# FengDushuo/BBBP-Multi-Modal-Deep-Ensemble-Framework

Hardware: AMD Instinct MI355X
Metric: molecules/sec fwd+bwd (3-branch ensemble, B=512) (higher is better)
Workload: dtype f32; 1 GPU; MixedInputModel F=167 (MACCS) + 3x128x128 image, 6-layer encoder + 2-stage CNN + fusion + BN head; forward + MSE + backward + fused AdamW, train mode (dropout 0.1); global_batch=512, per_gpu_batch=512, parallelism=dp1, input=device-resident

## Files before the change

### bbbp-multi-modal-deep-ensemble-framework_amd/_lib.py

```python
from __future__ import annotations

import ctypes
import os
import re
from ctypes import (POINTER, Structure, c_char_p, c_double, c_float, c_int, c_long, c_size_t, c_uint8, c_uint64, c_void_p)

_HERE = os.path.dirname(os.path.abspath(__file__))
LIB_PATH = os.environ.get("BBBP_LIB", os.path.join(_HERE, "libbbbp_hip.so"))
HEADER_PATH = os.path.join(os.path.dirname(_HERE), "include", "bbbp_hip.h")

_lib = None


class MixedDesc(Structure):
    _fields_ = [("batch", c_int), ("fingerprint_size", c_int), ("nhead", c_int), ("num_layers", c_int),
                ("dim_feedforward", c_int), ("training", c_int), ("dropout_p", c_float), ("seed", c_uint64),
                ("need_input_grad", c_int), ("fusion", c_int), ("inference", c_int),
                ("world", c_int), ("rank", c_int), ("collective", c_void_p), ("collective_ctx", c_void_p)]


CollectiveFn = ctypes.CFUNCTYPE(c_int, c_void_p, c_int, c_int, c_int, ctypes.c_size_t, ctypes.c_size_t, ctypes.c_size_t, c_void_p)


class GemmDesc(Structure):
    _fields_ = [("transA", c_int), ("transB", c_int), ("M", c_int), ("N", c_int), ("K", c_int), ("alpha", c_float),
                ("A", c_void_p), ("lda", c_int), ("B", c_void_p), ("ldb", c_int), ("C", c_void_p), ("ldc", c_int),
                ("bias", c_void_p), ("residual", c_void_p), ("ldr", c_int), ("act", c_int),
                ("gate", c_void_p), ("ldg", c_int), ("gate_scale", c_float), ("batch", c_int),
                ("strideA", c_long), ("strideB", c_long), ("strideC", c_long), ("strideR", c_long), ("strideG", c_long),
                ("gate_after_residual", c_int), ("asum", c_void_p), ("drop_p", c_float), ("drop_seed", c_uint64)]


class MlpModel(Structure):
    _fields_ = [("n_layers", c_int), ("units", c_int * 5), ("activation", c_int), ("batch_size", c_int), ("n_train", c_int),
                ("n_iter_no_change", c_int), ("max_iter", c_int),
                ("lr_init", ctypes.c_double), ("alpha", ctypes.c_double), ("beta1", ctypes.c_double), ("beta2", ctypes.c_double),
                ("eps", ctypes.c_double), ("tol", ctypes.c_double),
                ("params", c_void_p), ("adam_m", c_void_p), ("adam_v", c_void_p), ("grads", c_void_p),
                ("act", c_void_p), ("delta", c_void_p), ("order", c_void_p), ("loss_curve", c_void_p),
                ("t", c_long), ("best_loss", ctypes.c_double), ("no_improve", c_int), ("n_iter", c_int), ("done", c_int)]


class GemmF64cDesc(Structure):
    _fields_ = [("layout", c_int), ("M", c_int), ("N", c_int), ("K", c_int),
                ("A", c_void_p), ("a_dtype", c_int), ("lda", c_long), ("B", c_void_p), ("b_dtype", c_int), ("ldb", c_long),
                ("a_shift", c_void_p), ("b_shift", c_void_p), ("row_scale", c_void_p),
                ("C", c_void_p), ("c_dtype", c_int), ("ldc", c_long), ("symmetric", c_int), ("split_k", c_int)]


class KnnDesc(Structure):
    _fields_ = [("m", c_int), ("n", c_int), ("d", c_int), ("k", c_int),
                ("Q", c_void_p), ("q_dtype", c_int), ("ldq", c_long), ("T", c_void_p), ("t_dtype", c_int), ("ldt", c_long),
                ("mu", c_void_p), ("q_norm", c_void_p), ("t_norm", c_void_p), ("dist", c_void_p), ("ind", c_void_p),
                ("exclude_self", c_int), ("slices", c_int)]


_FP = c_void_p
_PP = POINTER(c_void_p)

_SIGNATURES = {
    "bbbp_abi_version": (c_int, []),
    "bbbp_last_error": (c_char_p, []),
    "bbbp_gemm_workspace_bytes": (c_size_t, [c_int, c_int, c_int, c_int]),
    "bbbp_gemm_f32": (c_int, [c_void_p, c_int, c_int, c_int, c_int, c_int, c_float, _FP, c_int, _FP, c_int, _FP, c_int,
                              _FP, _FP, c_int, c_int, c_int, c_long, c_long, c_long, c_long, c_void_p, c_size_t]),
    "bbbp_gemm_folds_asum": (c_int, [c_int, c_int, c_int, c_int]),
    "bbbp_gemm_f32_grouped": (c_int, [c_void_p, POINTER(GemmDesc), c_int, c_void_p, c_size_t]),
    "bbbp_mixed_backward_wait_bucket": (c_int, [c_void_p, c_int]),
    "bbbp_mixed_backward_wait_released": (c_int, [c_void_p, c_int]),
    "bbbp_set_release_events": (c_int, [c_int]),
    "bbbp_mixed_bucket_param": (c_int, [POINTER(MixedDesc), c_int]),
    "bbbp_mixed_bucket_range": (c_int, [POINTER(MixedDesc), c_int, POINTER(c_int), POINTER(c_int)]),
    "bbbp_mixed_debug_ffn_gate": (c_int, [c_void_p, POINTER(MixedDesc), c_void_p, c_int, c_void_p]),
    "bbbp_mixed_debug_pool_mask": (c_int, [c_void_p, POINTER(MixedDesc), c_void_p, c_int, c_void_p]),
    "bbbp_set_graphs": (c_int, [c_int]),
    "bbbp_set_fused_head_bwd": (c_int, [c_int]),
    "bbbp_set_fused_encoder": (c_int, [c_int]),
    "bbbp_set_fold_outproj": (c_int, [c_int]),
    "bbbp_set_flash_attention": (c_int, [c_int]),
    "bbbp_set_gemm_split_bf16": (c_int, [c_int]),
    "bbbp_set_gemm_fold_reduce": (c_int, [c_int]),
    "bbbp_gemm_split_bf16_phases": (c_int, [POINTER(c_uint64)]),
    "bbbp_gbt_predict": (c_int, [c_void_p, c_void_p, c_long, c_int, c_void_p, c_void_p, c_void_p, c_void_p, c_void_p, c_void_p, c_int, c_float,
                         c_void_p, c_void_p]),
    "bbbp_oblivious_predict": (c_int, [c_void_p, c_void_p, c_long, c_int, c_void_p, c_void_p, c_void_p, c_void_p, c_void_p, c_void_p, c_int,
                               c_double, c_double, c_void_p, c_void_p]),
    "bbbp_linear_layernorm_supported": (c_int, [c_int, c_int, c_int]),
    "bbbp_linear_layernorm_fwd": (c_int, [c_void_p, c_void_p, c_int, c_void_p, c_void_p, c_void_p, c_int, c_void_p, c_int, c_void_p, c_int, c_void_p,
                                  c_void_p, c_void_p, c_void_p, c_int, c_int, c_int, c_float, c_float, c_uint64]),
    "bbbp_layernorm_linear_supported": (c_int, [c_int, c_int, c_int]),
    "bbbp_layernorm_linear_fwd": (c_int, [c_void_p, c_void_p, c_int, c_void_p, c_void_p, c_float, c_void_p, c_void_p, c_void_p, c_int, c_int, c_float,
                                  c_uint64, c_void_p, c_int, c_void_p, c_void_p, c_int, c_int, c_int]),
    "bbbp_forest_groups": (c_int, [c_int]),
    "bbbp_forest_predict": (c_int, [c_void_p, c_void_p, c_long, c_int, c_void_p, c_void_p, c_void_p, c_void_p, c_void_p, c_void_p, c_int,
                                    c_void_p, c_void_p]),
    "bbbp_mlp_train_epochs": (c_int, [c_void_p, c_void_p, c_int, c_void_p, c_void_p, c_int, c_int]),
    "bbbp_mlp_predict_proba": (c_int, [c_void_p, c_void_p, c_int, c_void_p, c_int, c_int, c_int, c_void_p]),
    "bbbp_pca_col_mean": (c_int, [c_void_p, c_void_p, c_int, c_long, c_int, c_long, c_void_p]),
    "bbbp_gemm_f64c_workspace_bytes": (c_size_t, [POINTER(GemmF64cDesc)]),
    "bbbp_gemm_f64c": (c_int, [c_void_p, POINTER(GemmF64cDesc), c_void_p, c_size_t]),
    "bbbp_knn_row_norms": (c_int, [c_void_p, c_void_p, c_int, c_long, c_int, c_long, c_void_p, c_void_p, c_void_p]),
    "bbbp_knn_workspace_bytes": (c_size_t, [POINTER(KnnDesc)]),
    "bbbp_knn_f64": (c_int, [c_void_p, POINTER(KnnDesc), c_void_p, c_size_t]),
    "bbbp_knn_vote": (c_int, [c_void_p, c_void_p, c_void_p, c_long, c_int, c_int, c_void_p, c_long, c_int, c_int, c_void_p, c_void_p]),
    "bbbp_graph_stats": (c_int, [POINTER(c_long), POINTER(c_long)]),
    "bbbp_conv_last_clock": (c_int, [POINTER(c_uint64), POINTER(c_uint64)]),
    "bbbp_set_conv_winograd": (c_int, [c_int]),
    "bbbp_get_conv_winograd": (c_int, []),
    "bbbp_conv_winograd_phases": (c_int, [POINTER(c_uint64)]),
    "bbbp_conv_b3_phases": (c_int, [POINTER(c_uint64)]),
    "bbbp_conv3x3_workspace_bytes": (c_size_t, [c_int, c_int, c_int, c_int, c_int]),
    "bbbp_conv3x3_relu_pool_fwd": (c_int, [c_void_p, _FP, _FP, _FP, _FP, c_void_p, c_int, c_int, c_int, c_int, c_int,
                                           c_void_p, c_size_t]),
    "bbbp_conv3x3_relu_pool_bwd_data": (c_int, [c_void_p, _FP, c_void_p, _FP, _FP, c_int, c_int, c_int, c_int, c_int,
                                                c_void_p, c_size_t]),
    "bbbp_conv3x3_relu_pool_bwd_weight": (c_int, [c_void_p, _FP, _FP, c_void_p, _FP, _FP, c_int, c_int, c_int, c_int,
                                                  c_int, c_void_p, c_size_t]),
    "bbbp_layernorm_fwd": (c_int, [c_void_p, _FP, _FP, _FP, _FP, _FP, _FP, _FP, c_int, c_int, c_float, c_float, c_uint64]),
    "bbbp_layernorm_bwd": (c_int, [c_void_p, _FP, _FP, _FP, _FP, _FP, _FP, _FP, _FP, _FP, c_int, c_int, c_float, c_uint64]),
    "bbbp_softmax_fwd": (c_int, [c_void_p, _FP, _FP, c_long, c_int, c_float, c_uint64]),
# ... 77 lines not shown
```

### bbbp-multi-modal-deep-ensemble-framework_amd/csrc/gemm.hip

```cpp
#include "common.h"
#include "bbbp_hip.h"
#include <mutex>
#include <type_traits>
#include <unordered_map>

#define TRY_RC(expr) do { int _rc = (expr); if (_rc) return _rc; } while (0)

typedef float f32x4u __attribute__((ext_vector_type(4), aligned(4)));
typedef float f32x2u __attribute__((ext_vector_type(2), aligned(4)));

namespace {

constexpr int bk_of(int tile) { return tile == 64 ? 16 : 32; }

struct GemmParams {
    const float* A; const float* B; float* C;
    const float* bias; const float* R;
    int M, N, K;
    int lda, ldb, ldc, ldr;
    long sA, sB, sC, sR;
    float alpha;
    int act;
    int splits, kchunk;
    float* slab;
// ... 237 lines not shown
            step = B3_BK;
        }
    }
    __device__ __forceinline__ void load(int set) {
#pragma unroll
        for (int i = 0; i < 4; ++i) { raw[set][i] = *reinterpret_cast<const f32x4u*>(ptr[i]); ptr[i] += step; }
        kpos += B3_BK;
    }
    __device__ __forceinline__ void load_tail(int set) {
        if constexpr (KMAJ) {
#pragma unroll
            for (int j = 0; j < 4; ++j) {
                const bool ok = kpos + j < kend;
                const f32x4u v = *reinterpret_cast<const f32x4u*>(ok ? ptr[j] : X0);
                raw[set][j] = ok ? v : f32x4u{0.f, 0.f, 0.f, 0.f};
            }
        } else {
            const int nv = kend - kpos;
#pragma unroll
            for (int i = 0; i < 4; ++i) {
                const float* q = nv > 0 ? ptr[i] : X0;
                f32x4u v;
#pragma unroll
                for (int e = 0; e < 4; ++e) { const float x = q[e < nv ? e : 0]; v[e] = e < nv ? x : 0.f; }
                raw[set][i] = v;
            }
        }
        kpos += B3_BK;
    }
    __device__ __forceinline__ void split(int set) {
#pragma unroll
        for (int i = 0; i < 4; ++i) {
            uint32_t h0, m0, l0, h1, m1, l1;
            if constexpr (KMAJ) {
                split2(raw[set][0][i], raw[set][1][i], h0, m0, l0);
                split2(raw[set][2][i], raw[set][3][i], h1, m1, l1);
            } else {
                split2(raw[set][i][0], raw[set][i][1], h0, m0, l0);
                split2(raw[set][i][2], raw[set][i][3], h1, m1, l1);
            }
            pk[i][0] = u32x2{h0, h1}; pk[i][1] = u32x2{m0, m1}; pk[i][2] = u32x2{l0, l1};
        }
    }
    __device__ __forceinline__ void store(uint16_t* dst) const {
#pragma unroll
        for (int i = 0; i < 4; ++i)
#pragma unroll
            for (int pl = 0; pl < 3; ++pl) *reinterpret_cast<u32x2*>(dst + soff[i] + pl * B3_PLANE) = pk[i][pl];
    }
};

__device__ unsigned long long g_gemm_b3_phase[7];

template <int LAYOUT, bool PROBE>
__device__ __forceinline__ void gemm_b3_body(const GemmParams& p) {
    BBBP_HIGH_PRIO();
    unsigned long long ph[5] = {0, 0, 0, 0, 0}, c0 = 0;
    const unsigned long long cyc_begin = PROBE ? __builtin_readcyclecounter() : 0, wall_begin = PROBE ? wall_clock64() : 0;
    constexpr bool A_KMAJ = (LAYOUT == 2), B_KMAJ = (LAYOUT != 0);
    extern __shared__ __attribute__((aligned(16))) uint16_t smem16[];
    uint16_t* As = smem16;
    uint16_t* Bs = smem16 + 3 * B3_PLANE;
    const int t = threadIdx.x, lane = t & 63, wave = t >> 6, r = lane & 31, h = lane >> 5;
    const int wm = wave >> 1, wn = wave & 1;
    const int batch = blockIdx.z / p.splits, split = blockIdx.z % p.splits;
    const int m0 = blockIdx.y * 128, n0 = blockIdx.x * 128;
    const int kbeg = split * p.kchunk;
    const int kend = min(p.K, kbeg + p.kchunk);
    const int nt = (kend - kbeg + B3_BK - 1) / B3_BK;
    const int tail_stage = ((kend - kbeg) % B3_BK) ? nt - 1 : -1;

    B3Loader<A_KMAJ> la;
    B3Loader<B_KMAJ> lb;
    la.init(p.A + (long)batch * p.sA, p.lda, p.M, m0, kbeg, kend, t);
    lb.init(p.B + (long)batch * p.sB, p.ldb, p.N, n0, kbeg, kend, t);
    auto load_stage = [&](int stage, int set) __attribute__((always_inline)) {
        if (stage == tail_stage) { la.load_tail(set); lb.load_tail(set); }
        else { la.load(set); lb.load(set); }
    };

    f32x16 acc[2][2];
#pragma unroll
    for (int i = 0; i < 2; ++i)
#pragma unroll
        for (int j = 0; j < 2; ++j)
#pragma unroll
            for (int q = 0; q < 16; ++q) acc[i][j][q] = 0.f;

    if (nt > 0) {
        load_stage(0, 0);
        if (nt > 1) load_stage(1, 1);
        la.split(0); lb.split(0);
        la.store(As); lb.store(Bs);
    }
    __syncthreads();
    const uint16_t* afrag = As + (wm * 64 + r) * B3_LD + 8 * h;
    const uint16_t* bfrag = Bs + (wn * 64 + r) * B3_LD + 8 * h;
    for (int it = 0; it < nt; it += 2) {
#pragma unroll
        for (int u = 0; u < 2; ++u) {
            const int cur = it + u;
            if (cur >= nt) break;
            if (PROBE) c0 = __builtin_readcyclecounter();
            if (cur + 2 < nt) load_stage(cur + 2, u);
            if (PROBE) { const unsigned long long c = __builtin_readcyclecounter(); ph[0] += c - c0; c0 = c; }
#pragma unroll
// ... 44 lines not shown
#pragma unroll
            for (int j = 0; j < 2; ++j) {
                const int n = n0 + wn * 64 + j * 32 + r;
#pragma unroll
                for (int q = 0; q < 16; ++q) {
                    const int m = m0 + wm * 64 + i * 32 + mfma_row(q, lane);
                    if (m < p.M && n < p.N) {
                        if (p.arrivals) __hip_atomic_store(&S[(long)m * p.N + n], acc[i][j][q], __ATOMIC_RELAXED, __HIP_MEMORY_SCOPE_AGENT);
                        else S[(long)m * p.N + n] = acc[i][j][q];
                    }
                }
            }
        if (!p.arrivals) return;
        __shared__ int s_last;
        asm volatile("s_waitcnt vmcnt(0)" ::: "memory");
        __syncthreads();
        if (t == 0) {
            unsigned* cnt = p.arrivals + ((long)batch * gridDim.y + blockIdx.y) * gridDim.x + blockIdx.x;
            const unsigned old = __hip_atomic_fetch_add(cnt, 1u, __ATOMIC_RELAXED, __HIP_MEMORY_SCOPE_AGENT);
            s_last = (old == (unsigned)p.splits - 1u) ? 1 : 0;
            if (s_last) __hip_atomic_store(cnt, 0u, __ATOMIC_RELAXED, __HIP_MEMORY_SCOPE_AGENT);
        }
        __syncthreads();
        if (!s_last) return;
        const long mn = (long)p.M * p.N;
        const float* S0 = p.slab + (long)batch * p.splits * mn;
        float* Cf = p.C + (long)batch * p.sC;
        const float* Rf = p.R ? p.R + (long)batch * p.sR : nullptr;
        const int tw = min(128, p.N - n0), th = min(128, p.M - m0);
        for (int e = t; e < th * 128; e += 256) {
            const int lm = e >> 7, ln = e & 127;
            if (ln >= tw) continue;
            const int m = m0 + lm, n = n0 + ln;
            const float* sp = S0 + (long)m * p.N + n;
            float sum = 0.f;
            int k = 0;
            for (; k + 8 <= p.splits; k += 8) {
                float v[8];
#pragma unroll
                for (int u = 0; u < 8; ++u) v[u] = __hip_atomic_load(sp + (long)(k + u) * mn, __ATOMIC_RELAXED, __HIP_MEMORY_SCOPE_AGENT);
#pragma unroll
                for (int u = 0; u < 8; ++u) sum += v[u];
            }
            for (; k < p.splits; ++k) sum += __hip_atomic_load(sp + (long)k * mn, __ATOMIC_RELAXED, __HIP_MEMORY_SCOPE_AGENT);
            float v = apply_act(p.alpha * sum + (p.bias ? p.bias[n] : 0.f), p.act);
            const float gsel = p.gate ? (p.gate[(long)batch * p.sG + (long)m * p.ldg + n] > 0.f ? p.gate_scale : 0.f) : 1.f;
            if (!p.gate_after) v *= gsel;
            if (Rf) v += Rf[(long)m * p.ldr + n];
            if (p.gate_after) v *= gsel;
            Cf[(long)m * p.ldc + n] = v;
        }
        return;
    }
    float* C = p.C + (long)batch * p.sC;
    const float* R = p.R ? p.R + (long)batch * p.sR : nullptr;
#pragma unroll
    for (int i = 0; i < 2; ++i)
#pragma unroll
        for (int j = 0; j < 2; ++j) {
            const int n = n0 + wn * 64 + j * 32 + r;
            const float bv = (p.bias && n < p.N) ? p.bias[n] : 0.f;
#pragma unroll
            for (int q = 0; q < 16; ++q) {
                const int m = m0 + wm * 64 + i * 32 + mfma_row(q, lane);
                if (m < p.M && n < p.N) {
                    float v = apply_act(p.alpha * acc[i][j][q] + bv, p.act);
                    const float gsel = p.gate ? (p.gate[(long)batch * p.sG + (long)m * p.ldg + n] > 0.f ? p.gate_scale : 0.f) : 1.f;
                    if (!p.gate_after) v *= gsel;
                    if (R) v += R[(long)m * p.ldr + n];
                    if (p.gate_after) v *= gsel;
                    C[(long)m * p.ldc + n] = v;
                }
            }
        }
}

template <int LAYOUT>
__global__ __launch_bounds__(256, 2) void gemm_b3_kernel(GemmParams p) { gemm_b3_body<LAYOUT, false>(p); }
template <int LAYOUT>
__global__ __launch_bounds__(256, 2) void gemm_b3_probe_kernel(GemmParams p) { gemm_b3_body<LAYOUT, true>(p); }

constexpr int B3S_T = 64;
#ifndef BBBP_B3S_DEPTH_NT
#define BBBP_B3S_DEPTH_NT 2
#endif
#ifndef BBBP_B3S_DEPTH_NN
#define BBBP_B3S_DEPTH_NN 2
#endif
constexpr int B3S_DEPTH_NT = BBBP_B3S_DEPTH_NT, B3S_DEPTH_NN = BBBP_B3S_DEPTH_NN;
constexpr int B3S_PLANE = B3S_T * B3_LD;
constexpr size_t B3S_LDS = (size_t)6 * B3S_PLANE * sizeof(uint16_t);

template <bool KMAJ, int SETS>
struct B3SLoader {
    static constexpr int NL = KMAJ ? 4 : 2;
    const float* ptr[NL];
    const float* X0;
    long step;
    int kpos, kend;
    int soff[NL];
    bool live;
    f32x4u raw[SETS][NL];
    u32x2 pk[NL][3];
    __device__ __forceinline__ void init(const float* X, int ld, int extent, int row0, int kbeg, int kend_, int t) {
        const int kq = t & 7, rq = t >> 3;
        X0 = X; kpos = kbeg + 4 * kq; kend = kend_;
        if constexpr (KMAJ) {
            live = rq < 16;
            const int cq = rq & 15;
            const int col = min(row0 + 4 * cq, extent - 4);
#pragma unroll
            for (int j = 0; j < 4; ++j) { ptr[j] = X + (long)(kbeg + 4 * kq + j) * ld + col; soff[j] = (4 * cq + j) * B3_LD + 4 * kq; }
            step = (long)B3_BK * ld;
        } else {
            live = true;
            const int a = rq & 3, b = rq >> 2;
            const int row = (b >> 2) * 16 + (b & 3) + 4 * a;
#pragma unroll
            for (int i = 0; i < 2; ++i) {
                ptr[i] = X + (long)min(row0 + row + 32 * i, extent - 1) * ld + kbeg + 4 * kq;
                soff[i] = (row + 32 * i) * B3_LD + 4 * kq;
            }
            step = B3_BK;
        }
    }
    __device__ __forceinline__ void load(int set) {
#pragma unroll
        for (int i = 0; i < NL; ++i) { raw[set][i] = *reinterpret_cast<const f32x4u*>(ptr[i]); ptr[i] += step; }
        kpos += B3_BK;
    }
    __device__ __forceinline__ void load_tail(int set) {
        if constexpr (KMAJ) {
#pragma unroll
// ... 574 lines not shown
            }
        }
    }
    {
        float ta[4][1], tb[4][1];
        opa.fetch_tail(nch - 1, p.K, ta); opb.fetch_tail(nch - 1, p.K, tb);
        chunk(ta, tb, nch - 1, true);
    }
    s1 += __shfl_xor(s1, 16); s1 += __shfl_xor(s1, 32);
    s2 += __shfl_xor(s2, 16); s2 += __shfl_xor(s2, 32);
    cn += __shfl_xor(cn, 16); cn += __shfl_xor(cn, 32);
    dn += __shfl_xor(dn, 16); dn += __shfl_xor(dn, 32);
    const float mus = s1 / p.K;
    const float rstd = rsqrtf(fmaxf(s2 / p.K - mus * mus, 0.f) + p.eps);
    const int n = opb.index(0, q);
    const float bv = (p.bias && n < p.N) ? p.bias[n] : 0.f;
    const uint64_t seed = effective_seed(p.drop_seed, p.seed_base);
#pragma unroll
    for (int r = 0; r < 4; ++r) {
        const int m = opa.index(0, 4 * kq + r);
        const float mu_r = __shfl(mus, 4 * kq + r), rs_r = __shfl(rstd, 4 * kq + r);
        if (m < p.M && n < p.N) {
            float v = apply_act(rs_r * (acc[r] - mu_r * cn) + dn + bv, p.act);
            if (p.drop_p > 0.f) v *= dropout_scale(seed, (uint64_t)m * p.N + n, p.drop_p, p.drop_inv_keep);
            p.C[(long)m * p.ldc + n] = v;
        }
    }
}

template <int L0, int T0, int L1, int T1>
__global__ __launch_bounds__(256) void gemm_direct_pair_kernel(DirectParams p0, DirectParams p1) {
    BBBP_HIGH_PRIO();
    extern __shared__ float red[];
    if ((int)blockIdx.z < p0.batch) {
        if ((int)blockIdx.x < p0.gx && (int)blockIdx.y < p0.gy) gemm_direct_body<L0, T0, T0>(p0, blockIdx.z, red);
    } else {
        if ((int)blockIdx.x < p1.gx && (int)blockIdx.y < p1.gy) gemm_direct_body<L1, T1, T1>(p1, blockIdx.z - p0.batch, red);
    }
}



struct GemmKnobs {
    int direct;
    int direct_ks;
    int direct_t;
    int b3_small;
    int tall_b3;
    int split_x10;
    int split_full;
    int short_k, short_tiles;
    int reduce_vec4;
    int b3_probe;
    int split_bf16;
    int fold_reduce;
};
Knob g_gemm_b3{"BBBP_GEMM_SPLIT_BF16", 1, knob_bool};
Knob g_gemm_fold_reduce{"BBBP_GEMM_FOLD_REDUCE", 0, knob_bool};
GemmKnobs gemm_knobs() {
    static const GemmKnobs env{bbbp_env_int("BBBP_GEMM_DIRECT", 1), bbbp_env_int("BBBP_GEMM_DIRECT_KS", 2), bbbp_env_int("BBBP_GEMM_DIRECT_T", 2),
                               bbbp_env_int("BBBP_GEMM_B3_SMALL", 1), bbbp_env_int("BBBP_GEMM_TALL_B3", 1), bbbp_env_int("BBBP_GEMM_SPLIT_X10", 20),
                               bbbp_env_int("BBBP_GEMM_SPLIT_FULL", 0), bbbp_env_int("BBBP_GEMM_SHORT_K", 256), bbbp_env_int("BBBP_GEMM_SHORT_TILES", 4),
                               bbbp_env_int("BBBP_GEMM_REDUCE_VEC4", 1), bbbp_env_int("BBBP_GEMM_B3_PROBE", 0), 0, 0};
    GemmKnobs k = env;
    k.split_bf16 = g_gemm_b3.get();
    k.fold_reduce = g_gemm_fold_reduce.get();
    return k;
}

constexpr int ARRIVAL_REGION = 8192, ARRIVAL_REGIONS = 32;
unsigned* arrival_counters(hipStream_t st) {
    static std::mutex mu;
    static unsigned* base[64] = {};
    static std::unordered_map<hipStream_t, int> region[64];
    int dev = 0;
    if (hipGetDevice(&dev) != hipSuccess || dev < 0 || dev >= 64) return nullptr;
    std::lock_guard<std::mutex> lock(mu);
    if (!base[dev]) {
        hipStreamCaptureStatus cap = hipStreamCaptureStatusNone;
        (void)hipStreamIsCapturing(st, &cap);
        if (cap != hipStreamCaptureStatusNone) return nullptr;
        unsigned* ptr = nullptr;
        const size_t bytes = (size_t)ARRIVAL_REGION * ARRIVAL_REGIONS * sizeof(unsigned);
        if (hipMalloc(&ptr, bytes) != hipSuccess) return nullptr;
        if (hipMemset(ptr, 0, bytes) != hipSuccess || hipDeviceSynchronize() != hipSuccess) { (void)hipFree(ptr); return nullptr; }
        base[dev] = ptr;
    }
    auto it = region[dev].find(st);
    if (it == region[dev].end()) {
        if ((int)region[dev].size() >= ARRIVAL_REGIONS) return nullptr;
        it = region[dev].emplace(st, (int)region[dev].size()).first;
    }
    return base[dev] + (size_t)it->second * ARRIVAL_REGION;
}

constexpr int LAYOUT_ANY = -1;
struct GemmProblem {
    int M, N, K, batch;
    int layout = LAYOUT_ANY;
    bool asum_column = false;
    bool quad_epilogue = false;
};

enum class GemmKernel {
    Direct,
    B3Small,
    B3,
    F32Tile128,
    F32Tile128ShortK,
    F32Tile64
};
struct GemmPlan {
    GemmKernel kernel = GemmKernel::F32Tile64;
    int tile = 0, splits = 1, kchunk = 0;
    int t = 1, wsm = 1, wsn = 1, ks = 1;
    int gx = 0, gy = 0, gz = 0;
    size_t slab_bytes = 0;
    bool reduce = false, reduce_vec4 = false;
    bool in_kernel_reduce = false;
    bool asum_dropout = false;
};

GemmPlan gemm_plan(const GemmProblem& pr, int ncu, const GemmKnobs& kn, bool split_k = true) {
    const int M = pr.M, N = pr.N, K = pr.K, batch = pr.batch;
    GemmPlan pl;
    if (kn.direct && 2.0 * M * N * (double)K * batch <= 1.2e9 && K <= 8192) {
        const int nch = cdiv(K, 16);
        pl.ks = nch <= 12 ? 1 : (cdiv(nch, 8) < kn.direct_ks ? cdiv(nch, 8) : kn.direct_ks);
        if (pl.ks == 3) pl.ks = 4;
        const long wt = (long)cdiv(M, 16) * cdiv(N, 16) * batch;
        pl.t = (wt * pl.ks <= 4096 || kn.direct_t < 2) ? 1 : 2;
        const long waves = (long)cdiv(M, 16 * pl.t) * cdiv(N, 16 * pl.t) * batch * pl.ks;
        const int mind = M < N ? (M < K ? M : K) : (N < K ? N : K);
        if (pl.ks >= 4) { pl.wsm = 1; pl.wsn = 1; }
        else if (pl.ks >= 2) { pl.wsm = 2; pl.wsn = 1; }
        else { pl.wsm = 2; pl.wsn = 2; }
        if (waves <= 16384 && !(batch >= 8 && mind < 16) && !((kn.direct & 2) && pl.ks > 1) && !((kn.direct & 4) && pl.t > 1)) {
            pl.kernel = GemmKernel::Direct;
            pl.gx = cdiv(N + (pr.asum_column ? 1 : 0), 16 * pl.t * pl.wsn); pl.gy = cdiv(M, 16 * pl.t * pl.wsm); pl.gz = batch;
            pl.asum_dropout = true;
            return pl;
        }
        pl = GemmPlan{};
    }
    const long t128 = (long)cdiv(M, 128) * cdiv(N, 128) * batch, t64 = (long)cdiv(M, 64) * cdiv(N, 64) * batch;
    const long covered = (long)cdiv(M, 128) * 128 * (long)cdiv(N, 128) * 128;
    pl.tile = (t128 >= (long)ncu * 3 / 4) ? 128 : 64;
    if (K >= 8192 && M >= 128 && N >= 128) pl.tile = 128;
    if (K >= 512 && M >= 256 && N >= 256 && covered * 100 <= (long)M * N * 115) pl.tile = 128;
    if (kn.tall_b3 && K >= 1024 && M >= 1024 && N >= 128 && covered * 10 <= (long)M * N * 16) pl.tile = 128;
    const long tiles = pl.tile == 128 ? t128 : t64;
    const int BK = bk_of(pl.tile);
    int s = 1;
    if (split_k && (tiles < ncu || (kn.split_full && tiles < 2 * ncu && K >= 512)) && K >= 256) {
        s = (int)(((long)kn.split_x10 * ncu / 10 + tiles - 1) / tiles);
        if (s > K / 64) s = K / 64;
        if (s < 1) s = 1;
    }
    pl.kchunk = cdiv(cdiv(K, s), BK) * BK;
    if (pl.kchunk < BK) pl.kchunk = BK;
    pl.splits = cdiv(K, pl.kchunk) < 1 ? 1 : cdiv(K, pl.kchunk);
    pl.gx = cdiv(N, pl.tile); pl.gy = cdiv(M, pl.tile); pl.gz = batch * pl.splits;
    pl.slab_bytes = pl.splits > 1 ? (size_t)batch * pl.splits * M * N * sizeof(float) : 0;
    pl.reduce = pl.splits > 1;
    pl.reduce_vec4 = pl.reduce && kn.reduce_vec4 && N % 4 == 0 && pr.quad_epilogue;
    pl.kernel = pl.tile == 128 ? GemmKernel::F32Tile128 : GemmKernel::F32Tile64;
    if (pl.tile != 128 || pr.layout == LAYOUT_ANY) return pl;
    const bool b3 = kn.split_bf16 && K >= 32 && (pr.layout != 2 || (M % 4 == 0 && M >= 4)) && (pr.layout == 0 || (N % 4 == 0 && N >= 4));
    if (b3 && pr.layout != 2 && kn.b3_small && K >= 512 && t128 < ncu && t64 * 2 >= (long)ncu * 5) {
        pl.kernel = GemmKernel::B3Small;
        pl.splits = 1; pl.kchunk = cdiv(K, B3_BK) * B3_BK;
        pl.gx = cdiv(N, B3S_T); pl.gy = cdiv(M, B3S_T); pl.gz = batch;
        pl.slab_bytes = 0; pl.reduce = pl.reduce_vec4 = false;
    } else if (b3) {
        pl.kernel = GemmKernel::B3;
        pl.in_kernel_reduce = kn.fold_reduce && pl.splits > 1 && (long)pl.gx * pl.gy * batch <= ARRIVAL_REGION;
    } else {
        const bool vec = (pr.layout == 2 ? M : K) % 4 == 0 && (pr.layout == 0 ? K : N) % 4 == 0;
        if (vec && pl.splits == 1 && K <= kn.short_k && t128 >= (long)kn.short_tiles * ncu) pl.kernel = GemmKernel::F32Tile128ShortK;
    }
    return pl;
}

template <int... Vs, class F>
void with_constant(int v, F&& f) { (void)(... || (v == Vs ? (f(std::integral_constant<int, Vs>{}), true) : false)); }
#define CONST_OF(x) decltype(x)::value

inline size_t direct_lds(const DirectParams& p, int t) {
    const int waves = p.wsm * p.wsn * p.ks;
    size_t lds = p.ks > 1 ? (size_t)waves * t * t * 4 * 64 * sizeof(float) : 0;
    return lds < g_bbbp_small_lds_pad ? g_bbbp_small_lds_pad : lds;
}

void launch_direct(const DirectParams& p, int layout, int t, hipStream_t st) {
    with_constant<1, 2>(t, [&](auto T) { with_constant<0, 1, 2>(layout, [&](auto L) {
        hipLaunchKernelGGL((gemm_direct_kernel<CONST_OF(L), CONST_OF(T), CONST_OF(T)>), dim3(p.gx, p.gy, p.batch), dim3(64 * p.wsm * p.wsn * p.ks),
                           direct_lds(p, CONST_OF(T)), st, p);
    }); });
}

template <int L0, int T0, int L1, int T1>
void launch_pair_one(const DirectParams& a, const DirectParams& b, hipStream_t st) {
    const size_t la = direct_lds(a, T0), lb = direct_lds(b, T1);
    dim3 grid(a.gx > b.gx ? a.gx : b.gx, a.gy > b.gy ? a.gy : b.gy, a.batch + b.batch);
    hipLaunchKernelGGL((gemm_direct_pair_kernel<L0, T0, L1, T1>), grid, dim3(256), la > lb ? la : lb, st, a, b);
}

bool launch_pair(const DirectParams& a, int la, int ta, const DirectParams& b, int lb, int tb, hipStream_t st) {
    if (a.wsm * a.wsn * a.ks != 4 || b.wsm * b.wsn * b.ks != 4 || ta != 1 || tb != 1 || (long)a.batch + b.batch > 65535) return false;
    if (la == 2 && lb == 0) { launch_pair_one<2, 1, 0, 1>(a, b, st); return true; }
    if (la == 1 && lb == 2) { launch_pair_one<1, 1, 2, 1>(a, b, st); return true; }
    if (la == 2 && lb == 2) { launch_pair_one<2, 1, 2, 1>(a, b, st); return true; }
    return false;
}

template <int BM, int BN, int LAYOUT, bool VEC, int BKT = 0>
void launch_f32_tile(const GemmParams& p, dim3 grid, hipStream_t st) {
    constexpr int BK = BKT ? BKT : bk_of(BM);
    constexpr size_t lds = (size_t)2 * BK * ((BM + (LAYOUT == 2 ? 4 : 1)) + (BN + (LAYOUT != 0 ? 4 : 1))) * sizeof(float);
    if (lds > 64 * 1024) (void)bbbp_ensure_dyn_lds(reinterpret_cast<const void*>(gemm_f32_kernel<BM, BN, LAYOUT, VEC, BKT>), lds);
    hipLaunchKernelGGL((gemm_f32_kernel<BM, BN, LAYOUT, VEC, BKT>), grid, dim3(256), lds > g_bbbp_small_lds_pad ? lds : g_bbbp_small_lds_pad, st, p);
}

template <int LAYOUT>
int launch_b3(const GemmParams& p, dim3 grid, bool probe, hipStream_t st) {
    if (!probe) return launch_lds(gemm_b3_kernel<LAYOUT>, grid, 256, B3_LDS, st, p);
// ... 42 lines not shown
    d.gate = g.gate; d.ldg = g.ldg; d.sG = g.strideG; d.gate_scale = g.gate_scale; d.gate_after = g.gate_after_residual;
}

DirectParams direct_params(const bbbp_gemm_desc& g, const GemmProblem& pr, const GemmPlan& pl) {
    DirectParams d;
    copy_desc(d, g);
    d.wsm = pl.wsm; d.wsn = pl.wsn; d.ks = pl.ks;
    d.asum = pr.asum_column ? g.asum : nullptr;
    d.drop_p = g.drop_p; d.drop_inv_keep = g.drop_p > 0.f ? 1.f / (1.f - g.drop_p) : 1.f; d.drop_seed = g.drop_seed; d.seed_base = g_bbbp_seed_base;
    d.batch = pl.gz; d.gx = pl.gx; d.gy = pl.gy;
    return d;
}

GemmParams tile_params(const bbbp_gemm_desc& g, const GemmPlan& pl, void* workspace) {
    GemmParams p;
    copy_desc(p, g);
    p.vecA = ((g.transA ? g.M : g.K) % 4 == 0);
    p.vecB = ((g.transB ? g.K : g.N) % 4 == 0);
    p.splits = pl.splits; p.kchunk = pl.kchunk;
    p.slab = pl.slab_bytes ? static_cast<float*>(workspace) : nullptr;
    p.arrivals = nullptr;
    p.short_k = pl.kernel == GemmKernel::F32Tile128ShortK;
    return p;
}

int gemm_run(hipStream_t st, const bbbp_gemm_desc& g, void* workspace, size_t workspace_bytes) {
    TRY_RC(gemm_validate(g));
    if (g.M == 0 || g.N == 0) return BBBP_OK;
    const int ncu = bbbp_num_cus();
    const GemmKnobs kn = gemm_knobs();
    const GemmProblem pr = problem_of(g, workspace);
    GemmPlan pl = gemm_plan(pr, ncu, kn);
    if (pl.slab_bytes && (!workspace || workspace_bytes < pl.slab_bytes)) pl = gemm_plan(pr, ncu, kn, false);
    if (pl.kernel == GemmKernel::Direct) {
        launch_direct(direct_params(g, pr, pl), pr.layout, pl.t, st);
        BBBP_CHECK_LAUNCH();
        return BBBP_OK;
    }
    BBBP_CHECK_ARG(!g.asum, "gemm: asum is only produced by the small-product path (bbbp_gemm_folds_asum(%d, %d, %d, %d) == 0)", g.M, g.N, g.K, g.batch);
    BBBP_CHECK_ARG(!(g.drop_p > 0.f), "gemm: output dropout is only applied by the small-product path (bbbp_gemm_folds_asum(%d, %d, %d, %d) == 0)", g.M, g.N, g.K, g.batch);
    BBBP_CHECK_ARG(pl.gy <= 65535 && pl.gz <= 65535, "gemm: grid too large");
    GemmParams p = tile_params(g, pl, workspace);
    const dim3 grid(pl.gx, pl.gy, pl.gz);
    const bool vec = p.vecA && p.vecB;
    int rc = BBBP_OK;
    switch (pl.kernel) {
    case GemmKernel::B3Small:
        with_constant<0, 1>(pr.layout, [&](auto L) { rc = launch_b3_small<CONST_OF(L)>(p, grid, st); });
        break;
    case GemmKernel::B3:
        if (pl.in_kernel_reduce) p.arrivals = arrival_counters(st);
        with_constant<0, 1, 2>(pr.layout, [&](auto L) { rc = launch_b3<CONST_OF(L)>(p, grid, kn.b3_probe != 0, st); });
        break;
    case GemmKernel::F32Tile128ShortK:
        with_constant<0, 1, 2>(pr.layout, [&](auto L) { launch_f32_tile<128, 128, CONST_OF(L), true, 16>(p, grid, st); });
        break;
    case GemmKernel::F32Tile128:
        with_constant<0, 1, 2>(pr.layout, [&](auto L) { with_constant<1, 0>(vec, [&](auto V) { launch_f32_tile<128, 128, CONST_OF(L), CONST_OF(V) != 0>(p, grid, st); }); });
        break;
    default:
        with_constant<0, 1, 2>(pr.layout, [&](auto L) { with_constant<1, 0>(vec, [&](auto V) { launch_f32_tile<64, 64, CONST_OF(L), CONST_OF(V) != 0>(p, grid, st); }); });
    }
    TRY_RC(rc);
    BBBP_CHECK_LAUNCH();
    if (pl.reduce && !p.arrivals) {
        const long quads = ((long)g.M * g.N / (pl.reduce_vec4 ? 4 : 1) + 255) / 256;
        const dim3 rgrid((unsigned)(quads > 4096 ? 4096 : quads), g.batch);
        if (pl.reduce_vec4) hipLaunchKernelGGL(gemm_splitk_reduce4_kernel, rgrid, dim3(256), g_bbbp_small_lds_pad, st, p);
        else hipLaunchKernelGGL(gemm_splitk_reduce_kernel, rgrid, dim3(256), g_bbbp_small_lds_pad, st, p);
        BBBP_CHECK_LAUNCH();
    }
    return BBBP_OK;
}

GemmPlan gemm_plan_any_layout(int M, int N, int K, int batch) { return gemm_plan(GemmProblem{M, N, K, batch}, bbbp_num_cus(), gemm_knobs()); }

}

extern "C" int bbbp_gemm_folds_asum(int M, int N, int K, int batch) {
    return (M > 0 && N > 0 && K > 0 && batch >= 1 && gemm_plan_any_layout(M, N, K, batch).asum_dropout) ? 1 : 0;
}

extern "C" size_t bbbp_gemm_workspace_bytes(int M, int N, int K, int batch) {
    return (M <= 0 || N <= 0) ? 0 : gemm_plan_any_layout(M, N, K, batch).slab_bytes;
}

extern "C" int bbbp_gemm_f32(void* stream, int transA, int transB, int M, int N, int K, float alpha,
                             const float* A, int lda, const float* B, int ldb, float* C, int ldc,
                             const float* bias, const float* residual, int ldr, int act,
                             int batch, long strideA, long strideB, long strideC, long strideR,
                             void* workspace, size_t workspace_bytes) {
    bbbp_gemm_desc g;
    g.transA = transA; g.transB = transB; g.M = M; g.N = N; g.K = K; g.alpha = alpha;
    g.A = A; g.lda = lda; g.B = B; g.ldb = ldb; g.C = C; g.ldc = ldc;
    g.bias = bias; g.residual = residual; g.ldr = ldr; g.act = act;
    g.gate = nullptr; g.ldg = 0; g.gate_scale = 1.f; g.gate_after_residual = 0; g.asum = nullptr; g.drop_p = 0.f; g.drop_seed = 0;
    g.batch = batch; g.strideA = strideA; g.strideB = strideB; g.strideC = strideC; g.strideR = strideR; g.strideG = 0;
    return gemm_run(static_cast<hipStream_t>(stream), g, workspace, workspace_bytes);
}

extern "C" int bbbp_gemm_f32_grouped(void* stream, const bbbp_gemm_desc* problems, int count, void* workspace,
                                     size_t workspace_bytes) {
    BBBP_CHECK_ARG(count >= 0 && (count == 0 || problems), "gemm_grouped: bad arguments");
    hipStream_t st = static_cast<hipStream_t>(stream);
    int i = 0;
    while (i < count) {
        if (i + 1 < count) {
            const bbbp_gemm_desc &a = problems[i], &b = problems[i + 1];
            TRY_RC(gemm_validate(a));
            TRY_RC(gemm_validate(b));
            if (a.M > 0 && a.N > 0 && b.M > 0 && b.N > 0) {
                const int ncu = bbbp_num_cus();
                const GemmKnobs kn = gemm_knobs();
                const GemmProblem pa = problem_of(a, workspace), pb = problem_of(b, workspace);
                const GemmPlan la = gemm_plan(pa, ncu, kn), lb = gemm_plan(pb, ncu, kn);
                if (la.kernel == GemmKernel::Direct && lb.kernel == GemmKernel::Direct &&
                    launch_pair(direct_params(a, pa, la), pa.layout, la.t, direct_params(b, pb, lb), pb.layout, lb.t, st)) {
                    BBBP_CHECK_LAUNCH();
                    i += 2;
                    continue;
                }
            }
        }
        TRY_RC(gemm_run(st, problems[i], workspace, workspace_bytes));
        ++i;
    }
    return BBBP_OK;
}

extern "C" int bbbp_set_gemm_fold_reduce(int on) { return g_gemm_fold_reduce.set(on); }

extern "C" int bbbp_set_gemm_split_bf16(int on) { return g_gemm_b3.set(on); }


extern "C" int bbbp_gemm_split_bf16_phases(unsigned long long* phases7) {
    BBBP_CHECK_ARG(phases7 != nullptr, "gemm_split_bf16_phases: null output");
    BBBP_CHECK_HIP(hipDeviceSynchronize());
// ... 56 lines not shown
```

### include/bbbp_hip.h

```cpp
#ifndef BBBP_HIP_H
#define BBBP_HIP_H

#include <stddef.h>
#include <stdint.h>

#ifdef __cplusplus
extern "C" {
#endif

#define BBBP_OK 0
#define BBBP_ERR_ARG 1
#define BBBP_ERR_HIP 2
#define BBBP_ERR_WORKSPACE 3

#define BBBP_ACT_NONE 0
#define BBBP_ACT_RELU 1
#define BBBP_ACT_TANH 2

int bbbp_abi_version(void);
const char* bbbp_last_error(void);

size_t bbbp_gemm_workspace_bytes(int M, int N, int K, int batch);
int bbbp_gemm_f32(void* stream, int transA, int transB, int M, int N, int K, float alpha,
                  const float* A, int lda, const float* B, int ldb, float* C, int ldc,
                  const float* bias, const float* residual, int ldr, int act,
                  int batch, long strideA, long strideB, long strideC, long strideR,
                  void* workspace, size_t workspace_bytes);

typedef struct bbbp_gemm_desc {
    int transA, transB, M, N, K;
    float alpha;
    const float* A; int lda;
    const float* B; int ldb;
    float* C; int ldc;
    const float* bias;
    const float* residual; int ldr;
    int act;
    const float* gate; int ldg; float gate_scale;
    int batch;
    long strideA, strideB, strideC, strideR, strideG;
    int gate_after_residual;
    float* asum;
    float drop_p;
    unsigned long long drop_seed;
} bbbp_gemm_desc;
int bbbp_gemm_folds_asum(int M, int N, int K, int batch);
int bbbp_gemm_f32_grouped(void* stream, const bbbp_gemm_desc* problems, int count, void* workspace, size_t workspace_bytes);

size_t bbbp_conv3x3_workspace_bytes(int B, int cin, int cout, int H, int W);
int bbbp_conv_last_clock(unsigned long long* shader_cycles, unsigned long long* ticks_100mhz);
int bbbp_set_conv_winograd(int mask);
int bbbp_get_conv_winograd(void);
int bbbp_conv_winograd_phases(unsigned long long* phases4);
int bbbp_conv_b3_phases(unsigned long long* phases4);
int bbbp_conv3x3_relu_pool_fwd(void* stream, const float* x, const float* w, const float* bias,
                               float* y, uint8_t* mask, int B, int cin, int cout, int H, int W,
                               void* workspace, size_t workspace_bytes);
int bbbp_conv3x3_relu_pool_bwd_data(void* stream, const float* gy, const uint8_t* mask, const float* w,
                                    float* dx, int B, int cin, int cout, int H, int W,
                                    void* workspace, size_t workspace_bytes);
int bbbp_conv3x3_relu_pool_bwd_weight(void* stream, const float* x, const float* gy, const uint8_t* mask,
                                      float* dw, float* db, int B, int cin, int cout, int H, int W,
                                      void* workspace, size_t workspace_bytes);

int bbbp_layernorm_fwd(void* stream, float* x_inout_z, const float* residual, float* y, const float* gamma,
                       const float* beta, float* mean, float* rstd, int rows, int cols, float eps,
                       float dropout_p, uint64_t seed);
int bbbp_linear_layernorm_supported(int M, int N, int K);
int bbbp_linear_layernorm_fwd(void* stream, const float* x, int ldx, const float* W, const float* bias, const float* residual, int ldr,
                              float* z, int ldz, float* y, int ldy, const float* gamma, const float* beta, float* mean, float* rstd,
                              int M, int N, int K, float eps, float dropout_p, uint64_t seed);
int bbbp_layernorm_linear_supported(int M, int N, int K);
int bbbp_layernorm_linear_fwd(void* stream, const float* z, int ldz, const float* gamma, const float* beta, float eps,
                              const float* W, const float* bias, float* out, int ldo, int act, float dropout_p, uint64_t seed,
                              float* y, int ldy, float* mean, float* rstd, int M, int N, int K);
int bbbp_layernorm_bwd(void* stream, const float* dy, const float* z, const float* gamma, const float* mean,
                       const float* rstd, float* dz, float* dx, float* dgamma, float* dbeta, int rows, int cols,
                       float dropout_p, uint64_t seed);

int bbbp_softmax_fwd(void* stream, float* x_inout, float* dropped_out, long rows, int cols, float dropout_p,
                     uint64_t seed);
int bbbp_softmax_bwd(void* stream, float* dprob_inout, const float* prob, long rows, int cols, float dropout_p,
                     uint64_t seed);

int bbbp_dropout(void* stream, const float* x, float* y, long n, float p, uint64_t seed);

int bbbp_batchnorm1d_fwd(void* stream, const float* x, float* y, const float* gamma, const float* beta,
                         float* running_mean, float* running_var, float* save_mean, float* save_rstd, int rows,
                         int cols, float eps, float momentum, int training);
int bbbp_batchnorm1d_bwd(void* stream, const float* dy, const float* x, const float* gamma, const float* save_mean,
                         const float* save_rstd, float* dx, float* dgamma, float* dbeta, int rows, int cols,
                         int training);
int bbbp_batchnorm1d_bwd_relu(void* stream, const float* dy, const float* x, const float* gamma, const float* save_mean,
                         const float* save_rstd, float* dx, float* dgamma, float* dbeta, int rows, int cols,
                         int training);

int bbbp_column_moments(void* stream, const float* x, const float* centre, float* sum_out, float* sumsq_out, int rows, int cols);
int bbbp_batchnorm1d_bwd_apply(void* stream, const float* dy, const float* x, const float* gamma, const float* mean,
                               const float* rstd, const float* sum_dy, const float* sum_dy_xhat, float* dx, int rows,
                               int cols, long n_global);
// ... 167 lines not shown
```

Measured before the change: 216,700 molecules/s.

## Add B-resident split-bf16 GEMM kernel that sweeps M tiles with LDS-resident B

Adds a GEMM kernel for short-K (K<=128) layouts that loads the whole 128-column B panel into LDS once, as three bf16 split planes. Each block then loops over every M tile, streaming A and writing one epilogue per tile. The goal is to avoid reloading and resplitting B for each output tile and to cut launch width for tall-M problems. The epilogue is factored out with a fast path that has no gate or residual. Selection is gated so that by default it only triggers when N/128 reaches the CU count. Using one block per CU with a large LDS footprint lowers occupancy.

```diff
diff --git a/bbbp-multi-modal-deep-ensemble-framework_amd/_lib.py b/bbbp-multi-modal-deep-ensemble-framework_amd/_lib.py
--- a/bbbp-multi-modal-deep-ensemble-framework_amd/_lib.py
+++ b/bbbp-multi-modal-deep-ensemble-framework_amd/_lib.py
@@ -66,6 +66,7 @@
                               _FP, _FP, c_int, c_int, c_int, c_long, c_long, c_long, c_long, c_void_p, c_size_t]),
     "bbbp_gemm_folds_asum": (c_int, [c_int, c_int, c_int, c_int]),
     "bbbp_gemm_f32_grouped": (c_int, [c_void_p, POINTER(GemmDesc), c_int, c_void_p, c_size_t]),
+    "bbbp_gemm_kernel_form": (c_int, [c_int, c_int, c_int, c_int, c_int, c_int]),
     "bbbp_mixed_backward_wait_bucket": (c_int, [c_void_p, c_int]),
     "bbbp_mixed_backward_wait_released": (c_int, [c_void_p, c_int]),
     "bbbp_set_release_events": (c_int, [c_int]),
diff --git a/bbbp-multi-modal-deep-ensemble-framework_amd/csrc/gemm.hip b/bbbp-multi-modal-deep-ensemble-framework_amd/csrc/gemm.hip
--- a/bbbp-multi-modal-deep-ensemble-framework_amd/csrc/gemm.hip
+++ b/bbbp-multi-modal-deep-ensemble-framework_amd/csrc/gemm.hip
@@ -313,6 +313,56 @@
 
 __device__ unsigned long long g_gemm_b3_phase[7];
 
+__device__ __forceinline__ void b3_tile_epilogue(const GemmParams& p, const f32x16 (&acc)[2][2], int batch, int m0, int n0, int wm, int wn, int lane) {
+    const int r = lane & 31;
+    float* C = p.C + (long)batch * p.sC;
+    const float* R = p.R ? p.R + (long)batch * p.sR : nullptr;
+    if (!p.gate && !R) {
+        float bv[2];
+#pragma unroll
+        for (int j = 0; j < 2; ++j) {
+            const int n = n0 + wn * 64 + j * 32 + r;
+            bv[j] = (p.bias && n < p.N) ? p.bias[n] : 0.f;
+        }
+        asm volatile("" : "+v"(bv[0]), "+v"(bv[1]));
+        auto store_all = [&](auto plain) __attribute__((always_inline)) {
+#pragma unroll
+            for (int i = 0; i < 2; ++i)
+#pragma unroll
+                for (int j = 0; j < 2; ++j) {
+                    const int n = n0 + wn * 64 + j * 32 + r;
+#pragma unroll
+                    for (int q = 0; q < 16; ++q) {
+                        const int m = m0 + wm * 64 + i * 32 + mfma_row(q, lane);
+                        if (m < p.M && n < p.N) C[(long)m * p.ldc + n] = apply_act(p.alpha * acc[i][j][q] + bv[j], decltype(plain)::value ? 0 : p.act);
+                    }
+                }
+        };
+        if (p.act == 0) store_all(std::true_type{});
+        else store_all(std::false_type{});
+        return;
+    }
+#pragma unroll
+    for (int i = 0; i < 2; ++i)
+#pragma unroll
+        for (int j = 0; j < 2; ++j) {
+            const int n = n0 + wn * 64 + j * 32 + r;
+            const float bv = (p.bias && n < p.N) ? p.bias[n] : 0.f;
+#pragma unroll
+            for (int q = 0; q < 16; ++q) {
+                const int m = m0 + wm * 64 + i * 32 + mfma_row(q, lane);
+                if (m < p.M && n < p.N) {
+                    float v = apply_act(p.alpha * acc[i][j][q] + bv, p.act);
+                    const float gsel = p.gate ? (p.gate[(long)batch * p.sG + (long)m * p.ldg + n] > 0.f ? p.gate_scale : 0.f) : 1.f;
+                    if (!p.gate_after) v *= gsel;
+                    if (R) v += R[(long)m * p.ldr + n];
+                    if (p.gate_after) v *= gsel;
+                    C[(long)m * p.ldc + n] = v;
+                }
+            }
+        }
+}
+
 template <int LAYOUT, bool PROBE>
 __device__ __forceinline__ void gemm_b3_body(const GemmParams& p) {
     BBBP_HIGH_PRIO();
@@ -463,33 +513,120 @@
         }
         return;
     }
-    float* C = p.C + (long)batch * p.sC;
-    const float* R = p.R ? p.R + (long)batch * p.sR : nullptr;
-#pragma unroll
-    for (int i = 0; i < 2; ++i)
-#pragma unroll
-        for (int j = 0; j < 2; ++j) {
-            const int n = n0 + wn * 64 + j * 32 + r;
-            const float bv = (p.bias && n < p.N) ? p.bias[n] : 0.f;
-#pragma unroll
-            for (int q = 0; q < 16; ++q) {
-                const int m = m0 + wm * 64 + i * 32 + mfma_row(q, lane);
-                if (m < p.M && n < p.N) {
-                    float v = apply_act(p.alpha * acc[i][j][q] + bv, p.act);
-                    const float gsel = p.gate ? (p.gate[(long)batch * p.sG + (long)m * p.ldg + n] > 0.f ? p.gate_scale : 0.f) : 1.f;
-                    if (!p.gate_after) v *= gsel;
-                    if (R) v += R[(long)m * p.ldr + n];
-                    if (p.gate_after) v *= gsel;
-                    C[(long)m * p.ldc + n] = v;
-                }
-            }
-        }
+    b3_tile_epilogue(p, acc, batch, m0, n0, wm, wn, lane);
 }
 
 template <int LAYOUT>
 __global__ __launch_bounds__(256, 2) void gemm_b3_kernel(GemmParams p) { gemm_b3_body<LAYOUT, false>(p); }
 template <int LAYOUT>
 __global__ __launch_bounds__(256, 2) void gemm_b3_probe_kernel(GemmParams p) { gemm_b3_body<LAYOUT, true>(p); }
+
+constexpr int B3R_LD = 128 + 8;
+constexpr int B3R_PLANE = 128 * B3R_LD;
+constexpr size_t B3R_LDS = (size_t)3 * (B3R_PLANE + B3_PLANE) * sizeof(uint16_t);
+
+__global__ __launch_bounds__(256, 1) void gemm_b3r_kernel(GemmParams p) {
+    BBBP_HIGH_PRIO();
+    extern __shared__ __attribute__((aligned(16))) uint16_t smem16[];
+    uint16_t* Bs = smem16;
+    uint16_t* As = smem16 + 3 * B3R_PLANE;
+    const int t = threadIdx.x, lane = t & 63, wave = t >> 6, r = lane & 31, h = lane >> 5;
+    const int wm = wave >> 1, wn = wave & 1;
+    const int n0 = blockIdx.x * 128;
+    const int nt = p.K / B3_BK;
+    const int stages = nt * ((p.M + 127) / 128);
+
+    B3Loader<false> la;
+    int ld_s = 0, ld_m0 = 0;
+    la.init(p.A, p.lda, p.M, 0, 0, p.K, t);
+    auto load_a = [&](int set) __attribute__((always_inline)) {
+        if (ld_s == nt) { ld_s = 0; ld_m0 += 128; la.init(p.A, p.lda, p.M, ld_m0, 0, p.K, t); }
+        la.load(set);
+        ++ld_s;
+    };
+    load_a(0);
+    if (stages > 1) load_a(1);
+    {
+        B3Loader<true> lb;
+        lb.init(p.B, p.ldb, p.N, n0, 0, p.K, t);
+        const int kq = t & 7, rq = t >> 3;
+        lb.load(0);
+        if (nt > 1) lb.load(1);
+#pragma unroll
+        for (int s = 0; s < 128 / B3_BK; ++s) {
+            if (s >= nt) break;
+            lb.split(s & 1);
+            if (s + 2 < nt) lb.load(s & 1);
+#pragma unroll
+            for (int i = 0; i < 4; ++i)
+#pragma unroll
+                for (int pl = 0; pl < 3; ++pl)
+                    *reinterpret_cast<u32x2*>(Bs + pl * B3R_PLANE + (4 * rq + i) * B3R_LD + s * B3_BK + 4 * kq) = lb.pk[i][pl];
+        }
+    }
+    la.split(0);
+    la.store(As);
+    __syncthreads();
+
+    f32x16 acc[2][2];
+#pragma unroll
+    for (int i = 0; i < 2; ++i)
+#pragma unroll
+        for (int j = 0; j < 2; ++j)
+#pragma unroll
+            for (int q = 0; q < 16; ++q) acc[i][j][q] = 0.f;
+    const uint16_t* afrag = As + (wm * 64 + r) * B3_LD + 8 * h;
+    const uint16_t* bfrag = Bs + (wn * 64 + r) * B3R_LD + 8 * h;
+    int s = 0, m0 = 0;
+    for (int g0 = 0; g0 < stages; g0 += 2) {
+#pragma unroll
+        for (int u = 0; u < 2; ++u) {
+            const int g = g0 + u;
+            if (g >= stages) break;
+            if (g + 2 < stages) load_a(u);
+#pragma unroll
+            for (int kk = 0; kk < B3_BK / 16; ++kk) {
+                bf16x8 a[2][3], b[2][3];
+#pragma unroll
+                for (int i = 0; i < 2; ++i)
+#pragma unroll
+                    for (int pl = 0; pl < 3; ++pl) {
+                        a[i][pl] = *reinterpret_cast<const bf16x8*>(afrag + pl * B3_PLANE + i * 32 * B3_LD + kk * 16);
+                        b[i][pl] = *reinterpret_cast<const bf16x8*>(bfrag + pl * B3R_PLANE + i * 32 * B3R_LD + s * B3_BK + kk * 16);
+                    }
+                constexpr int PA[6] = {1, 2, 0, 1, 0, 0}, PB[6] = {1, 0, 2, 0, 1, 0};
+#pragma unroll
+                for (int q = 0; q < 6; ++q)
+#pragma unroll
+                    for (int i = 0; i < 2; ++i)
+#pragma unroll
+                        for (int j = 0; j < 2; ++j)
+                            acc[i][j] = __builtin_amdgcn_mfma_f32_32x32x16_bf16(a[i][PA[q]], b[j][PB[q]], acc[i][j], 0, 0, 0);
+            }
+            la.split(u ^ 1);
+#pragma unroll
+            for (int q = 0; q < 48; ++q) {
+                __builtin_amdgcn_sched_group_barrier(0x008, 1, 0);
+                __builtin_amdgcn_sched_group_barrier(0x002, 2, 0);
+            }
+            __syncthreads();
+            if (g + 1 < stages) la.store(As);
+            if (s == nt - 1) {
+                b3_tile_epilogue(p, acc, 0, m0, n0, wm, wn, lane);
+#pragma unroll
+                for (int i = 0; i < 2; ++i)
+#pragma unroll
+                    for (int j = 0; j < 2; ++j)
+#pragma unroll
+                        for (int q = 0; q < 16; ++q) acc[i][j][q] = 0.f;
+                s = 0; m0 += 128;
+            } else {
+                ++s;
+            }
+            __syncthreads();
+        }
+    }
+}
 
 constexpr int B3S_T = 64;
 #ifndef BBBP_B3S_DEPTH_NT
@@ -1170,6 +1307,7 @@
     int short_k, short_tiles;
     int reduce_vec4;
     int b3_probe;
+    int b_resident;
     int split_bf16;
     int fold_reduce;
 };
@@ -1179,7 +1317,7 @@
     static const GemmKnobs env{bbbp_env_int("BBBP_GEMM_DIRECT", 1), bbbp_env_int("BBBP_GEMM_DIRECT_KS", 2), bbbp_env_int("BBBP_GEMM_DIRECT_T", 2),
                                bbbp_env_int("BBBP_GEMM_B3_SMALL", 1), bbbp_env_int("BBBP_GEMM_TALL_B3", 1), bbbp_env_int("BBBP_GEMM_SPLIT_X10", 20),
                                bbbp_env_int("BBBP_GEMM_SPLIT_FULL", 0), bbbp_env_int("BBBP_GEMM_SHORT_K", 256), bbbp_env_int("BBBP_GEMM_SHORT_TILES", 4),
-                               bbbp_env_int("BBBP_GEMM_REDUCE_VEC4", 1), bbbp_env_int("BBBP_GEMM_B3_PROBE", 0), 0, 0};
+                               bbbp_env_int("BBBP_GEMM_REDUCE_VEC4", 1), bbbp_env_int("BBBP_GEMM_B3_PROBE", 0), bbbp_env_int("BBBP_GEMM_B_RESIDENT", 1), 0, 0};
     GemmKnobs k = env;
     k.split_bf16 = g_gemm_b3.get();
     k.fold_reduce = g_gemm_fold_reduce.get();
@@ -1221,12 +1359,13 @@
 };
 
 enum class GemmKernel {
-    Direct,
-    B3Small,
-    B3,
-    F32Tile128,
-    F32Tile128ShortK,
-    F32Tile64
+    Direct = 0,
+    B3Small = 1,
+    B3 = 2,
+    F32Tile128 = 3,
+    F32Tile128ShortK = 4,
+    F32Tile64 = 5,
+    B3Resident = 6
 };
 struct GemmPlan {
     GemmKernel kernel = GemmKernel::F32Tile64;
@@ -1242,7 +1381,9 @@
 GemmPlan gemm_plan(const GemmProblem& pr, int ncu, const GemmKnobs& kn, bool split_k = true) {
     const int M = pr.M, N = pr.N, K = pr.K, batch = pr.batch;
     GemmPlan pl;
-    if (kn.direct && 2.0 * M * N * (double)K * batch <= 1.2e9 && K <= 8192) {
+    const bool resident_shape = pr.layout == 1 && kn.split_bf16 && K >= B3_BK && K <= 128 && K % B3_BK == 0 && N % 128 == 0 && M >= 256 && batch == 1;
+    const bool resident_any_size = resident_shape && (kn.b_resident & 2);
+    if (kn.direct && !resident_any_size && 2.0 * M * N * (double)K * batch <= 1.2e9 && K <= 8192) {
         const int nch = cdiv(K, 16);
         pl.ks = nch <= 12 ? 1 : (cdiv(nch, 8) < kn.direct_ks ? cdiv(nch, 8) : kn.direct_ks);
         if (pl.ks == 3) pl.ks = 4;
@@ -1267,6 +1408,7 @@
     if (K >= 8192 && M >= 128 && N >= 128) pl.tile = 128;
     if (K >= 512 && M >= 256 && N >= 256 && covered * 100 <= (long)M * N * 115) pl.tile = 128;
     if (kn.tall_b3 && K >= 1024 && M >= 1024 && N >= 128 && covered * 10 <= (long)M * N * 16) pl.tile = 128;
+    if (resident_any_size) pl.tile = 128;
     const long tiles = pl.tile == 128 ? t128 : t64;
     const int BK = bk_of(pl.tile);
     int s = 1;
@@ -1290,6 +1432,9 @@
         pl.splits = 1; pl.kchunk = cdiv(K, B3_BK) * B3_BK;
         pl.gx = cdiv(N, B3S_T); pl.gy = cdiv(M, B3S_T); pl.gz = batch;
         pl.slab_bytes = 0; pl.reduce = pl.reduce_vec4 = false;
+    } else if (b3 && resident_shape && (kn.b_resident & 1) && (resident_any_size || N / 128 >= ncu)) {
+        pl.kernel = GemmKernel::B3Resident;
+        pl.gx = N / 128; pl.gy = 1; pl.gz = 1;
     } else if (b3) {
         pl.kernel = GemmKernel::B3;
         pl.in_kernel_reduce = kn.fold_reduce && pl.splits > 1 && (long)pl.gx * pl.gy * batch <= ARRIVAL_REGION;
@@ -1438,6 +1583,9 @@
         if (pl.in_kernel_reduce) p.arrivals = arrival_counters(st);
         with_constant<0, 1, 2>(pr.layout, [&](auto L) { rc = launch_b3<CONST_OF(L)>(p, grid, kn.b3_probe != 0, st); });
         break;
+    case GemmKernel::B3Resident:
+        rc = launch_lds(gemm_b3r_kernel, grid, 256, B3R_LDS, st, p);
+        break;
     case GemmKernel::F32Tile128ShortK:
         with_constant<0, 1, 2>(pr.layout, [&](auto L) { launch_f32_tile<128, 128, CONST_OF(L), true, 16>(p, grid, st); });
         break;
@@ -1469,6 +1617,12 @@
 
 extern "C" size_t bbbp_gemm_workspace_bytes(int M, int N, int K, int batch) {
     return (M <= 0 || N <= 0) ? 0 : gemm_plan_any_layout(M, N, K, batch).slab_bytes;
+}
+
+extern "C" int bbbp_gemm_kernel_form(int transA, int transB, int M, int N, int K, int batch) {
+    if (M <= 0 || N <= 0 || K <= 0 || batch < 1 || (transA && transB)) return -1;
+    const GemmProblem pr{M, N, K, batch, transA ? 2 : (transB ? 0 : 1)};
+    return (int)gemm_plan(pr, bbbp_num_cus(), gemm_knobs()).kernel;
 }
 
 extern "C" int bbbp_gemm_f32(void* stream, int transA, int transB, int M, int N, int K, float alpha,
diff --git a/include/bbbp_hip.h b/include/bbbp_hip.h
--- a/include/bbbp_hip.h
+++ b/include/bbbp_hip.h
@@ -46,6 +46,7 @@
 } bbbp_gemm_desc;
 int bbbp_gemm_folds_asum(int M, int N, int K, int batch);
 int bbbp_gemm_f32_grouped(void* stream, const bbbp_gemm_desc* problems, int count, void* workspace, size_t workspace_bytes);
+int bbbp_gemm_kernel_form(int transA, int transB, int M, int N, int K, int batch);
 
 size_t bbbp_conv3x3_workspace_bytes(int B, int cin, int cout, int H, int W);
 int bbbp_conv_last_clock(unsigned long long* shader_cycles, unsigned long long* ticks_100mhz);
```

Measured after the change: 220,600 molecules/s (median of 6 runs). 1.8% higher.
